# HandH1998/QQQ

Hardware: AMD Instinct MI355X
Metric: W4A8 GEMM TOPS + speedup vs fp16, M in {1..4096} N=8192 K=21760 (higher is better)
Workload: dtype i8 x i4 -> i32 -> f16; 1 GPU; qqq_gemm per-channel sweep M in {1,16,128,1024,4096} N=8192 K=21760 (configs[1]); step = the 5 calls; weights=12 rotating 89 MB int4 buffers (cold Infinity Cache), GPTQ-style N(0,0.02^2), launch=hipGraph replay, 1-step opener then 10 steps/graph, parallelism=single GPU

## Files before the change

qqq_amd/csrc/qqq_w4a8.hip:

```cpp

#include <map>
#include <mutex>
#include <thread>
#include <tuple>
#include <type_traits>
#include <utility>
#include <vector>

#include "qqq_common.hip.h"
#include "qqq_stream.hip.h"
#include "qqq_column.hip.h"
#include "qqq_panel.hip.h"
#include "qqq_tiled.hip.h"
#include "qqq_wide.hip.h"
#include "qqq_small.hip.h"
#include "qqq_act.hip.h"
#include "../../include/qqq_amd_act.h"
#include "qqq_attn.hip.h"
#include "../../include/qqq_amd_attn.h"
#include "qqq_decode.hip.h"
#include "../../include/qqq_amd_decode.h"
#include "qqq_kv8.hip.h"
#include "../../include/qqq_amd_kv8.h"
#include "qqq_paged.hip.h"
// ... 139 lines not shown
extern "C" int qqq_w4a8_model_us(int prob_m, int prob_n, int prob_k, int groupsize, int max_par, double* out) {
  g_err[0] = 0;
  if (!out || prob_m <= 0 || prob_n <= 0 || prob_k <= 0 || (prob_n % 64) != 0 || (prob_k % 64) != 0) {
    snprintf(g_err, sizeof(g_err), "qqq_w4a8_model_us: bad argument");
    return QQQ_ERR_ARG;
  }
  model_us(plan_ctx(prob_m, prob_n, prob_k, groupsize != -1, 256, max_par, true, true), out);
  return QQQ_OK;
}

extern "C" int qqq_w4a8_gemm_ex(const void* A, const void* B, void* C, void* D, const void* s1,
                                const void* s2, const void* s3, int prob_m, int prob_n, int prob_k,
                                void* workspace, int groupsize, int dev, void* stream, int thread_k,
                                int thread_n, int sms, int max_par, const qqq_tune_t* tune,
                                int32_t* acc_out, const void* bias) {
  return qqq_w4a8_gemm_ex2(A, B, C, D, s1, s2, s3, prob_m, prob_n, prob_k, workspace, groupsize, dev, stream, thread_k, thread_n, sms, max_par,
                           tune, acc_out, bias, nullptr);
}

extern "C" int qqq_w4a8_gemm_ex2(const void* A, const void* B, void* C, void* D, const void* s1,
                                 const void* s2, const void* s3, int prob_m, int prob_n, int prob_k,
                                 void* workspace, int groupsize, int dev, void* stream, int thread_k,
                                 int thread_n, int sms, int max_par, const qqq_tune_t* tune,
                                 int32_t* acc_out, const void* bias, const void* W8) {
  g_err[0] = 0;
  const int rc = ref_shape_check(prob_m, prob_n, prob_k, groupsize, thread_k, thread_n);
  if (rc != QQQ_OK) return rc;
  if (prob_m == 0 || prob_n == 0 || prob_k == 0) return QQQ_OK;
  if (!A || !B || !D || !s1 || !s2 || (groupsize != -1 && !s3)) {
    snprintf(g_err, sizeof(g_err), "null pointer argument");
    return QQQ_ERR_ARG;
  }
  if ((((uintptr_t)A | (uintptr_t)B | (uintptr_t)C | (uintptr_t)D | (uintptr_t)bias | (uintptr_t)acc_out |
        (groupsize != -1 ? (uintptr_t)s3 : 0)) & 15) != 0 ||
      (((uintptr_t)s2) & 7) != 0 || (((uintptr_t)s1 | (uintptr_t)workspace) & 3) != 0 || (((uintptr_t)W8) & 15) != 0) {
    snprintf(g_err, sizeof(g_err), "misaligned pointer argument (A/B/C/D/s3/bias/acc_out/W8: 16 bytes, s2: 8, s1/workspace: 4)");
    return QQQ_ERR_ARG;
  }
  const bool grouped = groupsize != -1;
  qqq_tune_t t;
  memset(&t, 0, sizeof(t));
  if (tune) t = *tune;
  t.w8 = (W8 != nullptr && t.w8 >= 0) ? 1 : -1;
  const int M = prob_m, N = prob_n, K = prob_k;
  int cur_dev = dev;
  if (dev < 0) (void)hipGetDevice(&cur_dev);
  const int cus_dev = device_cus_of(cur_dev);
  const bool capped = sms > 0 && sms < cus_dev;
  const PlanCtx ctx = plan_ctx(M, N, K, grouped, capped ? masked_cus(sms) : cus_dev, max_par, C != nullptr, workspace != nullptr);
  if (handoff_env_flags() & 4) t.fused |= 16;
  double est = -1.0;
  const Plan pl = make_plan(ctx, t, &est);
  if (const int M0 = choose_split(ctx, t, pl, est)) {
    qqq_tune_t tn = t;
    tn.split_m = -1;
    const int rc0 = qqq_w4a8_gemm_ex2(A, B, C, D, s1, s2, s3, M0, N, K, workspace, groupsize, dev, stream, thread_k, thread_n, sms, max_par, &tn,
                                      acc_out, bias, W8);
    if (rc0 != QQQ_OK) return rc0;
    return qqq_w4a8_gemm_ex2(static_cast<const int8_t*>(A) + (size_t)M0 * K, B, C, static_cast<_Float16*>(D) + (size_t)M0 * N,
                             static_cast<const float*>(s1) + M0, s2, s3, M - M0, N, K, workspace, groupsize, dev, stream, thread_k, thread_n, sms,
                             max_par, &tn, acc_out ? acc_out + (size_t)M0 * N : nullptr, bias, W8);
  }

  LaunchArgs a;
  a.A = static_cast<const int8_t*>(A);
  a.B = static_cast<const unsigned char*>(B);
  a.C = static_cast<int32_t*>(C);
  a.D = static_cast<_Float16*>(D);
  a.s1 = static_cast<const float*>(s1);
  a.s2 = static_cast<const float*>(s2);
  a.s3 = static_cast<const _Float16*>(s3);
  a.acc_out = acc_out;
  a.bias = static_cast<const _Float16*>(bias);
  a.tickets = static_cast<int*>(workspace);
  a.M = M;
  a.N = N;
  a.K = K;
  a.cus = ctx.cus;
  a.stream = static_cast<hipStream_t>(stream);
  a.skew = pl.skew;
  a.hflags = (pl.kernel == 2 || pl.kernel == 4 || pl.kernel == 5) ? ((t.fused >> 2) & (pl.kernel == 4 ? 15 : 7)) : 0;
  if (pl.kernel == 5 && pl.exch) a.hflags |= 8;
  if (pl.kernel == 5 && (t.fused & 128)) a.hflags |= 16;

  DeviceGuard guard(dev);
  hipError_t e = hipSuccess;
  bool reduce_launch;
  if ((pl.kernel == 1 || pl.kernel == 3 || pl.kernel == 4) && (M + 16 * pl.mt - 1) / (16 * pl.mt) > 65535) {
    snprintf(g_err, sizeof(g_err), "m=%d exceeds the grid of the small-m kernels (forced by tune)", M);
    return QQQ_ERR_ARG;
  }
  MaskedFork mf;
  if (capped) {
    hipStreamCaptureStatus cap = hipStreamCaptureStatusNone;
    if (hipStreamIsCapturing(a.stream, &cap) != hipSuccess) cap = hipStreamCaptureStatusNone;
    if (cap == hipStreamCaptureStatusNone) {
      MaskedStream* ms = masked_stream(cur_dev, sms, cus_dev, a.stream);
      if (!ms) {
        snprintf(g_err, sizeof(g_err), "sms=%d: could not create a CU-masked stream", sms);
        return QQQ_ERR_HIP;
      }
      mf.lock = std::unique_lock<std::mutex>(ms->mu);
      if ((e = hipEventRecord(ms->fork, a.stream)) != hipSuccess || (e = hipStreamWaitEvent(ms->s, ms->fork, 0)) != hipSuccess)
        return fail_hip(e, "fork into the CU-masked stream");
      mf.ms = ms;
      mf.caller = a.stream;
      a.stream = ms->s;
    }
  }
  if (pl.kernel == 5) {
    if (pl.w8) a.B = static_cast<const unsigned char*>(W8);
    e = launch_wide(a, pl.w8 ? 2 : (grouped ? 1 : 0), pl.mt, pl.bm, pl.pf, pl.pw, pl.ksplit, pl.chain != 0);
    if (e != hipSuccess) return fail_hip(e, "qqq_wide_kernel launch");
    reduce_launch = false;
  } else if (pl.kernel == 4) {
    e = launch_panel(a, grouped, pl.mt, pl.bm, pl.waves, pl.pw, pl.pf, pl.stages, pl.ksplit);
    if (e != hipSuccess) return fail_hip(e, "qqq_panel_kernel launch");
    reduce_launch = false;
  } else if (pl.kernel == 3) {
    e = launch_column(a, grouped, pl.mt, pl.pf, pl.ksplit, pl.waves);
    if (e != hipSuccess) return fail_hip(e, "qqq_column_kernel launch");
    reduce_launch = pl.ksplit > 1;
  } else if (pl.kernel == 1) {
    e = launch_stream(a, grouped, pl.mt, pl.waves, pl.pf, pl.ksplit | ((pl.fused == 3 && pl.ksplit > 1 ? pl.skew & 0xff : 0) << 16),
                      pl.ksplit > 1 ? (pl.fused == 1 ? 1 : (pl.fused == 3 ? 3 : 0)) : 0);
    if (e != hipSuccess) return fail_hip(e, "qqq_stream_kernel launch");
    reduce_launch = pl.ksplit > 1 && pl.fused != 1 && pl.fused != 3;
  } else {
    e = launch_tiled(a, grouped, pl.bm, pl.stages, pl.ksplit, pl.nslots, pl.pw);
    if (e != hipSuccess) return fail_hip(e, "qqq_tiled_kernel launch");
    reduce_launch = pl.ksplit > 1 && pl.nslots == 0;
  }
  if (reduce_launch) {
    const long long items = (long long)M * (N / 4);
    const int blocks = (int)((items + 63) / 64 > 8192 ? 8192 : (items + 63) / 64);
    hipLaunchKernelGGL(qqq_reduce_kernel, dim3(blocks), dim3(64), 0, a.stream, a.C, a.D, a.s1, a.s2,
                       a.acc_out, a.bias, M, N, pl.ksplit);
    e = hipGetLastError();
    if (e != hipSuccess) return fail_hip(e, "qqq_reduce_kernel launch");
  }
  if ((e = mf.join()) != hipSuccess) return fail_hip(e, "join from the CU-masked stream");
  return QQQ_OK;
}

extern "C" int qqq_w4a8_gemm(const void* A, const void* B, void* C, void* D, const void* s1,
                             const void* s2, const void* s3, int prob_m, int prob_n, int prob_k,
                             void* workspace, int groupsize, int dev, void* stream, int thread_k,
                             int thread_n, int sms, int max_par) {
  return qqq_w4a8_gemm_ex(A, B, C, D, s1, s2, s3, prob_m, prob_n, prob_k, workspace, groupsize, dev,
                          stream, thread_k, thread_n, sms, max_par, nullptr, nullptr, nullptr);
}

template <template <int, int> class Launch, typename... Args>
static int act_launch(const char* what, int m, int k, hipStream_t st, Args... args) {
  const int nvec = k / 8;
  const int vpt = (nvec + 255) / 256;
  if ((m <= 512 || nvec > 2048) && vpt > 2) {
    const int v4 = (nvec + 1023) / 1024;
    if (v4 <= 2)
      Launch<2, 1024>::run(m, st, args...);
    else if (v4 <= 4)
      Launch<4, 1024>::run(m, st, args...);
    else
      Launch<8, 1024>::run(m, st, args...);
  } else if (vpt <= 2)
    Launch<2, 256>::run(m, st, args...);
// ... 938 lines not shown
```

qqq_amd/csrc/qqq_wide.hip.h:

```cpp
#ifndef QQQ_AMD_QQQ_WIDE_HIP_H_
#define QQQ_AMD_QQQ_WIDE_HIP_H_


#ifndef QQQ_WIDE_ABLATE
#define QQQ_WIDE_ABLATE 0
#endif
#ifdef QQQ_PANEL_TRACE
#define QQQ_WTRV(i, v)                                                                                   \
  do {                                                                                                   \
    if (wn == 0 && qqq_trace_buf) qqq_trace_buf[(size_t)blockIdx.x * 16 + (i)] = (unsigned long long)(v); \
  } while (0)
#define QQQ_WTR(i) QQQ_WTRV(i, wall_clock64())
#else
#define QQQ_WTR(i) do {} while (0)
#define QQQ_WTRV(i, v) do {} while (0)
#endif
template <int... S, class F>
__device__ __forceinline__ void qqq_static_for(std::integer_sequence<int, S...>, F&& f) {
  (f(std::integral_constant<int, S>{}), ...);
}
template <int N, class F>
__device__ __forceinline__ void qqq_static_for(F&& f) {
  qqq_static_for(std::make_integer_sequence<int, N>{}, static_cast<F&&>(f));
}
// ... 78 lines not shown
__host__ __device__ constexpr int wide_bal_cost(int mode, int w) { return w == 0 ? 1 : (mode == 1 ? 2 : 1); }
__host__ __device__ constexpr int wide_bal_before(int mode, int mt, int hw, int t, int k, int cursors) {
  const int nslot = 2 * hw * mt, per = wide_bal_items(mode), ni = hw * per;
  int ct = 0, cb = 0, tc = 0;
  for (int j = 0; j < nslot; ++j) ct += wide_bal_cap(mode, mt, hw, t, j, cursors);
  for (int j = 0; j < k; ++j) cb += wide_bal_cap(mode, mt, hw, t, j, cursors);
  for (int i = 0; i < ni; ++i) tc += wide_bal_cost(mode, i % per);
  if (k >= nslot) return ni;
  int n = 0, e = 0;
  for (int i = 0; i < ni; ++i) {
    e += wide_bal_cost(mode, i % per);
    if ((long long)e * ct <= (long long)cb * tc) ++n;
  }
  return n;
}

template <int MODE, int MT, int HW, int T, int CURSORS>
struct WideBalTable {
  struct Tab {
    int before[2 * HW * MT + 1];
  };
  static constexpr Tab make() {
    Tab r{};
    constexpr int nslot = 2 * HW * MT, per = wide_bal_items(MODE), ni = HW * per;
    int cap[nslot] = {};
    int ct = 0, tc = 0;
    for (int j = 0; j < nslot; ++j) {
      cap[j] = wide_bal_cap(MODE, MT, HW, T, j, CURSORS);
      ct += cap[j];
    }
    for (int i = 0; i < ni; ++i) tc += wide_bal_cost(MODE, i % per);
    int cb = 0, n = 0, e = wide_bal_cost(MODE, 0);
    for (int k = 0; k < nslot; ++k) {
      while (n < ni && (long long)e * ct <= (long long)cb * tc) {
        ++n;
        if (n < ni) e += wide_bal_cost(MODE, n % per);
      }
      r.before[k] = n;
      cb += cap[k];
    }
    r.before[nslot] = ni;
    return r;
  }
  static constexpr Tab tab = make();
};

static_assert(WideBalTable<0, 16, 2, 0, 1>::tab.before[17] == wide_bal_before(0, 16, 2, 0, 17, 1) && WideBalTable<0, 16, 2, 1, 1>::tab.before[63] == wide_bal_before(0, 16, 2, 1, 63, 1) &&
                  WideBalTable<1, 8, 2, 1, 0>::tab.before[9] == wide_bal_before(1, 8, 2, 1, 9, 0) && WideBalTable<1, 16, 1, 0, 0>::tab.before[30] == wide_bal_before(1, 16, 1, 0, 30, 0),
              "the table is the function");

__host__ __device__ constexpr int wide_w8_refill_index(int mt, int hw, int k) {
  const int per = (2 * hw * mt) / (2 * hw);
  return k % per == 2 ? k / per : -1;
}
__host__ __device__ constexpr int wide_loads_in_slot(int mode, int mt, int hw, int t, int k) {
  int n = 0;
  if (mode == 1 && t == 1 && k == wide_scale_slot(hw) && !(QQQ_WIDE_ABLATE & 8)) n += 2;
  if (mode != 2 && wide_ring_load(mode, mt, hw, k) >= 0 && !(QQQ_WIDE_ABLATE & 8)) n += 1;
  if (mode == 2 && wide_w8_refill_index(mt, hw, k) >= 0 && !(QQQ_WIDE_ABLATE & 8)) n += 1;
  if (wide_dma_slot(mt, hw, k) && !(QQQ_WIDE_ABLATE & 2)) n += 1;
  return n;
}
__host__ __device__ constexpr int wide_loads_in_step(int mode, int mt, int hw, int t, int from, int to) {
  int n = 0;
  for (int k = from; k < to && k < 2 * hw * mt; ++k) n += wide_loads_in_slot(mode, mt, hw, t, k);
  return n;
}
__host__ __device__ constexpr int wide_loads_between(int mode, int mt, int hw, int t0, int k0, int steps, int k1) {
  int n = wide_loads_in_step(mode, mt, hw, t0, k0 + 1, 2 * hw * mt);
  for (int j = 1; j < steps; ++j) n += wide_loads_in_step(mode, mt, hw, (t0 + j) & 1, 0, 2 * hw * mt);
  return n + wide_loads_in_step(mode, mt, hw, (t0 + steps) & 1, 0, k1);
}
__host__ __device__ constexpr int wide_w8_last_refill_slot(int mt, int hw) {
  int last = 0;
  for (int k = 0; k < 2 * hw * mt; ++k) last = wide_w8_refill_index(mt, hw, k) >= 0 ? k : last;
  return last;
}
__host__ __device__ constexpr int wide_last_dma_slot(int mt, int hw) {
  int last = 0;
  for (int k = 0; k < 2 * hw * mt; ++k) last = wide_dma_slot(mt, hw, k) ? k : last;
  return last;
}

template <int MODE, int MT, int P, int RS, int HW, bool CHAIN = false>
__global__ __launch_bounds__(256) __attribute__((amdgpu_waves_per_eu(1, 1))) void qqq_wide_kernel(
    const int8_t* __restrict__ A, const unsigned char* __restrict__ B, int32_t* __restrict__ C, _Float16* __restrict__ D,
    const float* __restrict__ s1, const float* __restrict__ s2, const _Float16* __restrict__ s3,
    int32_t* __restrict__ acc_out, int* __restrict__ tickets, const _Float16* __restrict__ bias, const int M, const int N,
    const int K, const int tiles_m, const int tiles_n, const int PW, const int ksplit_hf) {
  const int ksplit = ksplit_hf & 0xffff, hflags = (ksplit_hf >> 16) & 0xff, skew = (ksplit_hf >> 24) & 0x3f;
  constexpr bool GROUPED = MODE == 1, W8 = MODE == 2;
  static_assert(MODE >= 0 && MODE <= 2, "0 per-channel, 1 per-group, 2 expanded int8");
  static_assert(!W8 || RS >= 3, "W8: a slot is refilled one step after its use -- RS - 1 steps of lead, the wait count needs at least one whole step in between");
  constexpr int RL = W8 ? RS - 1 : RS;
  static_assert(MT == 16 || MT == 8, "m-tiles of 16 tokens per wave (= per workgroup): 256 or 128 tokens");
  static_assert(HW == 2 || HW == 1, "a wave owns both 32-column halves of a 64-column group, or (128-column tiles) one");
  constexpr int ROWS = 16 * MT;
  constexpr int NQ = 2 * HW;
  constexpr int BN = 128 * HW;
  constexpr int NT = 256;
  constexpr int XB = ROWS * 128;
  constexpr int XPT = XB / 16 / NT;
  static_assert((2 * P) % RS == 0, "weight ring (in 64-k steps) must divide the unroll period");
  static_assert(P >= 4 && P <= 6, "LDS stage buffers: one being read, one complete, P - 2 in flight");
  constexpr int LA = P - 1;
  constexpr int NSLOT = NQ * MT;
  constexpr int EPR = HW == 2 ? 8 * MT : 16 * MT;
  constexpr int EP_STRIDE = BN + 4;

  extern __shared__ __attribute__((aligned(16))) unsigned char smem[];

  const int tid = threadIdx.x;
  const int lane = tid & 63;
  const int wn = __builtin_amdgcn_readfirstlane(tid >> 6);
  QQQ_WTR(0);

  int tile_m, tile_n, tile_lin, sp;
  auto locate = [&](const int lin, int& tm, int& tn) {
    const int full = (tiles_n / PW) * PW * tiles_m;
    if (lin < full) {
      const int panel = lin / (PW * tiles_m), within = lin % (PW * tiles_m);
      tm = within / PW;
      tn = panel * PW + within % PW;
    } else {
      const int rem = lin - full, pw = tiles_n % PW;
      tm = rem / pw;
      tn = (tiles_n / PW) * PW + rem % pw;
    }
  };
  int ch_first = 0, ch_stride = 0, ch_tiles = 1;
  {
    const int ntot = tiles_m * tiles_n * (CHAIN ? 1 : ksplit);
    const int bid = blockIdx.x;
    const int q = ntot >> 3, rr = ntot & 7;
    const int xcd = bid & 7, idx = bid >> 3;
    const int lin2 = (xcd < rr ? xcd * (q + 1) : rr * (q + 1) + (xcd - rr) * q) + idx;
    if constexpr (CHAIN) {
      const int cnt = q + (xcd < rr ? 1 : 0);
      ch_stride = (int)(gridDim.x >> 3);
      ch_first = lin2;
      ch_tiles = idx < cnt ? (cnt - idx + ch_stride - 1) / ch_stride : 0;
      if (ch_tiles == 0) return;
      sp = 0;
      tile_lin = lin2;
      locate(lin2, tile_m, tile_n);
    } else if (ksplit == 2 && (hflags & 16) != 0 && ((tiles_m * tiles_n) & 3) == 0) {
      const int per = (tiles_m * tiles_n) >> 2;
      sp = xcd & 1;
      tile_lin = (xcd >> 1) * per + idx;
      locate(tile_lin, tile_m, tile_n);
    } else {
      const int lin = lin2 / ksplit;
      sp = lin2 - lin * ksplit;
      tile_lin = lin;
      locate(lin, tile_m, tile_n);
    }
  }
  unsigned my_xcc = 0;
  if (!CHAIN && ksplit > 1) {
    asm volatile("s_getreg_b32 %0, hwreg(HW_REG_XCC_ID)" : "=s"(my_xcc));
    my_xcc &= 7u;
    if (tid == 0 && ksplit <= 6)
      __hip_atomic_fetch_or(tickets + 2 * (size_t)tile_lin, (int)((8u | my_xcc) << (8 + 4 * sp)), __ATOMIC_RELAXED, __HIP_MEMORY_SCOPE_AGENT);
  }
  const int mbase = tile_m * ROWS;
  const int ngroups = N >> 6;
  const int cb = tile_n * 4 + wn;
  int ng = HW == 2 ? cb : cb >> 1;
  const int whalf = HW == 2 ? 0 : (cb & 1);
  if (ng >= ngroups) ng = ngroups - 1;
  const unsigned rowbytes = (unsigned)N * 8u;
  const unsigned wstep = W8 ? (unsigned)N * 64u : 4u * rowbytes;
// ... 293 lines not shown
          else if constexpr (j >= 0) asm_load_w(wr[(sl + RS - 1) % RS][j], std::integral_constant<int, j>{}, swo);
        } else {
          constexpr int li = wide_dw_load_index(MT, HW, k);
          if constexpr (li >= 0) {
            if constexpr (CUR) asm_load_d(wq[sl][li / 4][li % 4], std::integral_constant<int, li>{}, cr_so, std::true_type{});
            else asm_load_d(wq[sl][li / 4][li % 4], std::integral_constant<int, li>{}, swo, std::false_type{});
          }
        }
      }
      constexpr int DP = wide_dma_period(MT, HW);
      if constexpr (wide_m0_slot(MT, HW, k) && !(QQQ_WIDE_ABLATE & 2))
        dma_m0(std::integral_constant<int, (u + LA) % P>{}, std::integral_constant<int, (XPT / 2) * t + k / DP>{});
      if constexpr (wide_dma_slot(MT, HW, k) && !(QQQ_WIDE_ABLATE & 2)) {
        if constexpr (CUR) dma_go_cur(std::integral_constant<int, (XPT / 2) * t + k / DP>{});
        else dma_go(std::integral_constant<int, (XPT / 2) * t + k / DP>{}, st_xso);
      }
      if constexpr (t == 1 && k == BSLOT) {
        constexpr int since = wide_loads_between(MODE, MT, HW, 1, wide_last_dma_slot(MT, HW), 2 * (P - 3), k + 1);
        static_assert(since < 64, "vmcnt is a 6-bit counter");
        if constexpr (!(QQQ_WIDE_ABLATE & 1)) asm volatile("s_waitcnt vmcnt(%0)\n\ts_barrier" : : "n"(since) : "memory");
        else asm volatile("s_waitcnt vmcnt(%0)" : : "n"(since) : "memory");
      }
      __builtin_amdgcn_sched_barrier(0);
    };
    qqq_static_for<NSLOT>(slot);
  };

  constexpr int SCB = ROWS * 4 + BN * 6;
  constexpr int SC0 = P * XB;
  const int cej = lane & 15, cecp = lane >> 4;
  const int cegrp = HW == 2 ? wn : (wn >> 1), cehalf = wn & 1;
  auto scale_dma = [&](const int tm, const int tn, const int par) __attribute__((always_inline)) {
    const unsigned voff = (unsigned)((64 * wn + lane) * 4);
    const int rows = M - tm * ROWS < ROWS ? M - tm * ROWS : ROWS, cols = N - tn * BN < BN ? N - tn * BN : BN;
    auto one = [&](const void* base, const unsigned bytes, const unsigned dst) {
      v4u d = descriptor(base);
      d[2] = (unsigned)__builtin_amdgcn_readfirstlane((int)bytes);
      const unsigned m0v = (unsigned)__builtin_amdgcn_readfirstlane((int)dst);
      asm volatile("s_mov_b32 m0, %2\n\ts_nop 4\n\tbuffer_load_dword %0, %1, 0 offen lds" : : "v"(voff), "s"(d), "s"(m0v) : "memory");
    };
    const unsigned r0 = (unsigned)(SC0 + par * SCB + 256 * wn);
    if (wn < ROWS / 64) one(s1 + (size_t)tm * ROWS, (unsigned)rows * 4u, r0);
    if (wn < BN / 64) one(s2 + (size_t)tn * BN, (unsigned)cols * 4u, r0 + ROWS * 4);
    if (wn < BN / 128 && bias) one(bias + (size_t)tn * BN, (unsigned)cols * 2u, r0 + ROWS * 4 + BN * 4);
  };
  auto flush_tile = [&](const int tm, const int tn, const int par) __attribute__((always_inline)) {
    asm volatile("s_nop 15\n\ts_nop 15" ::: "memory");
    const unsigned char* sc = smem + SC0 + par * SCB;
    const float* s1t = reinterpret_cast<const float*>(sc);
    const float* s2t = reinterpret_cast<const float*>(sc + ROWS * 4);
    const _Float16* bt = reinterpret_cast<const _Float16*>(sc + ROWS * 4 + BN * 4);
    const _Float16 nzc = (_Float16)-0.0f;
    const int cl = 64 * cegrp + 16 * cecp;
    const bool cols_ok = tn * BN + 64 * cegrp < N;
    float2 dsa[NQ], dsb[NQ];
    h4 dbv[NQ];
    int dl[NQ];
#pragma unroll
    for (int q = 0; q < NQ; ++q) {
      dl[q] = cl + 8 * (q & 1) + 4 * (HW == 2 ? (q >> 1) : cehalf);
      const int i0 = s2_stored_index(dl[q]);
      dsa[q] = *reinterpret_cast<const float2*>(s2t + i0);
      dsb[q] = *reinterpret_cast<const float2*>(s2t + i0 + 8);
      dbv[q] = (h4){nzc, nzc, nzc, nzc};
    }
    if (bias) {
#pragma unroll
      for (int q = 0; q < NQ; ++q) dbv[q] = *reinterpret_cast<const h4*>(bt + dl[q]);
    }
    v4i zero4 = {0, 0, 0, 0};
    asm volatile("" : "+v"(zero4));
    const int rows = M - tm * ROWS < ROWS ? M - tm * ROWS : ROWS;
    const __amdgpu_buffer_rsrc_t dview = __builtin_amdgcn_make_buffer_rsrc(D + (size_t)tm * ROWS * N, 0, rows * N * 2, 0x00020000);
    const __amdgpu_buffer_rsrc_t aview = __builtin_amdgcn_make_buffer_rsrc(acc_out ? acc_out + (size_t)tm * ROWS * N : (int32_t*)D, 0, rows * N * 4, 0x00020000);
    const unsigned drow = (unsigned)(cej * N + tn * BN) * 2u;
#pragma unroll
    for (int mt = 0; mt < MT; ++mt) {
      const float ts = s1t[16 * mt + cej];
      h4 o[NQ];
#pragma unroll
      for (int q = 0; q < NQ; q += 2) {
        v4i ra = acc[mt][q], rb = acc[mt][q + 1];
        asm volatile("" : "+v"(ra), "+v"(rb));
        asm volatile("v_mfma_i32_16x16x64_i8 %0, %1, %1, 0" : "+a"(acc[mt][q]) : "v"(zero4));
        asm volatile("v_mfma_i32_16x16x64_i8 %0, %1, %1, 0" : "+a"(acc[mt][q + 1]) : "v"(zero4));
        int a0 = ra[0], a1 = ra[1], a2 = ra[2], a3 = ra[3], b0 = rb[0], b1 = rb[1], b2 = rb[2], b3 = rb[3];
        asm volatile("s_nop 1\n\t"
                     "v_permlane16_swap_b32 %0, %1\n\tv_permlane16_swap_b32 %2, %3\n\t"
                     "v_permlane16_swap_b32 %4, %5\n\tv_permlane16_swap_b32 %6, %7\n\t"
                     "v_permlane32_swap_b32 %0, %2\n\tv_permlane32_swap_b32 %1, %3\n\t"
                     "v_permlane32_swap_b32 %4, %6\n\tv_permlane32_swap_b32 %5, %7"
                     : "+v"(a0), "+v"(a1), "+v"(a2), "+v"(a3), "+v"(b0), "+v"(b1), "+v"(b2), "+v"(b3));
        if (acc_out && cols_ok) {
          const unsigned ar = (drow + (unsigned)(16 * mt) * (unsigned)N * 2u) * 2u;
          __builtin_amdgcn_raw_buffer_store_b128((v4u){(unsigned)a0, (unsigned)a1, (unsigned)a2, (unsigned)a3}, aview, ar + (unsigned)dl[q] * 4u, 0, 0);
          __builtin_amdgcn_raw_buffer_store_b128((v4u){(unsigned)b0, (unsigned)b1, (unsigned)b2, (unsigned)b3}, aview, ar + (unsigned)dl[q + 1] * 4u, 0, 0);
        }
        o[q] = epilogue_vals4(a0, a1, a2, a3, ts, dsa[q], dsb[q]) + dbv[q];
        o[q + 1] = epilogue_vals4(b0, b1, b2, b3, ts, dsa[q + 1], dsb[q + 1]) + dbv[q + 1];
      }
      if (cols_ok) {
        const unsigned dr = drow + (unsigned)(16 * mt) * (unsigned)N * 2u;
        if constexpr (HW == 2) {
          const h8 lo8 = {o[0][0], o[0][1], o[0][2], o[0][3], o[2][0], o[2][1], o[2][2], o[2][3]};
          const h8 hi8 = {o[1][0], o[1][1], o[1][2], o[1][3], o[3][0], o[3][1], o[3][2], o[3][3]};
          __builtin_amdgcn_raw_buffer_store_b128(__builtin_bit_cast(v4u, lo8), dview, dr + (unsigned)cl * 2u, 0, 0);
          __builtin_amdgcn_raw_buffer_store_b128(__builtin_bit_cast(v4u, hi8), dview, dr + (unsigned)cl * 2u + 16u, 0, 0);
        } else {
          typedef unsigned v2u __attribute__((ext_vector_type(2)));
#pragma unroll
          for (int q = 0; q < NQ; ++q) __builtin_amdgcn_raw_buffer_store_b64(__builtin_bit_cast(v2u, o[q]), dview, dr + (unsigned)dl[q] * 2u, 0, 0);
        }
      }
      __builtin_amdgcn_sched_barrier(0);
    }
  };
  auto seam = [&]() __attribute__((always_inline)) {
    QQQ_WTRV(ch_pos < 7 ? 2 + 2 * ch_pos : 15, wall_clock64());
    flush_tile(cur_tm, cur_tn, ch_pos & 1);
    QQQ_WTRV(ch_pos < 7 ? 3 + 2 * ch_pos : 15, wall_clock64());
    ++ch_pos;
    cur_tm = nx_tm, cur_tn = nx_tn;
    cu_a_lo = nx_a_lo, cu_a_hi = nx_a_hi, cu_a_rec = nx_a_rec, cu_w_so = nx_w_so, cu_s_so = nx_s_so;
    if (ch_pos < ch_tiles) {
      scale_dma(cur_tm, cur_tn, ch_pos & 1);
      if (ch_pos + 1 < ch_tiles) locate(ch_first + (ch_pos + 1) * ch_stride, nx_tm, nx_tn);
      nx_tm = __builtin_amdgcn_readfirstlane(nx_tm), nx_tn = __builtin_amdgcn_readfirstlane(nx_tn);
      tile_ref(nx_tm, nx_tn, nx_a_lo, nx_a_hi, nx_a_rec, nx_w_so, nx_s_so);
    }
    cursors_at_stage0();
  };

  constexpr int RST = NT / (BN / 8);
  const int c8 = tid % (BN / 8), er0 = tid / (BN / 8);
  const int n = tile_n * BN + c8 * 8;
  float2 s2v[4] = {};
  const _Float16 nz = (_Float16)-0.0f;
  h8 bv = {nz, nz, nz, nz, nz, nz, nz, nz};
  if (!CHAIN && n < N) {
    const int i0s = s2_stored_index(n), i1s = s2_stored_index(n + 4);
    s2v[0] = *reinterpret_cast<const float2*>(s2 + i0s);
    s2v[1] = *reinterpret_cast<const float2*>(s2 + i0s + 8);
    s2v[2] = *reinterpret_cast<const float2*>(s2 + i1s);
    s2v[3] = *reinterpret_cast<const float2*>(s2 + i1s + 8);
    if (bias) bv = *reinterpret_cast<const h8*>(bias + n);
  }

  if constexpr (CHAIN) {
    scale_dma(tile_m, tile_n, 0);
    qqq_static_for<LA>([&](auto jc) { dma_stage_so(jc, (unsigned)decltype(jc)::value * 128u); });
#pragma unroll
    for (int j = 0; j < RL; ++j) {
      if constexpr (DW) load_d_step(cu_w_so + (unsigned)j * wstep, wq[j]);
      else load_w_so(cu_w_so + (unsigned)j * wstep, wr[j]);
    }
    if constexpr (GROUPED) {
#pragma unroll
      for (int j = 0; j < P; ++j) load_sc_so(cu_s_so + (unsigned)j * (unsigned)N * 2u, scr[j]);
    }
  } else {
    qqq_static_for<LA>([&](auto jc) { dma_stage(jc, decltype(jc)::value); });
#pragma unroll
    for (int j = 0; j < RL; ++j) {
      if constexpr (DW) load_d_step((unsigned)(2 * st0 + (j < KS ? j : KS - 1)) * wstep, wq[j]);
      else load_w(j, wr[j]);
    }
    if constexpr (GROUPED) {
#pragma unroll
      for (int j = 0; j < P; ++j) load_sc(j, scr[j]);
    }
  }
  qqq_static_for<RL>([&](auto jc) {
    constexpr int j = decltype(jc)::value;
    (void)wr[0];
    if constexpr (DW) {
      (void)wq[0][0][0];
      qqq_static_for<HW>([&](auto hfc) {
        constexpr int hf = decltype(hfc)::value;
        (void)wq[0][0][0];
        asm volatile("s_waitcnt vmcnt(0)" : "+v"(wq[j][hf][0]), "+v"(wq[j][hf][1]), "+v"(wq[j][hf][2]), "+v"(wq[j][hf][3]));
      });
    } else if constexpr (HW == 2) asm volatile("s_waitcnt vmcnt(0)" : "+v"(wr[j][0]), "+v"(wr[j][1]), "+v"(wr[j][2]), "+v"(wr[j][3]));
    else asm volatile("s_waitcnt vmcnt(0)" : "+v"(wr[j][0]), "+v"(wr[j][1]));
  });
  if constexpr (GROUPED) {
    qqq_static_for<P>([&](auto jc) {
      (void)scr[0];
      asm volatile("" : "+v"(scr[decltype(jc)::value][0]), "+v"(scr[decltype(jc)::value][1]));
    });
  }
  __syncthreads();
#pragma unroll
  for (int mt = 0; mt < MT; ++mt) read_x(0, 0, mt);
  if constexpr (!W8) {
    qqq_static_for<HW>([&](auto hfc) {
      constexpr int hf = decltype(hfc)::value;
      un_setup(__builtin_bit_cast(h2, scr[0][hf]));
      (void)wq[0][0][0];
      qqq_static_for<UPARTS>([&](auto pc) { un_part(pc, hfc, aop[0], wq[0][hf]); });
    });
  }
  __builtin_amdgcn_sched_barrier(0);

  if constexpr (CUR) {
    cx_so = sgpr((unsigned)(st0 + LA - 1) * 128u);
    cr_so = sgpr((unsigned)(2 * st0 + RL) * wstep);
    cc_so = sgpr((unsigned)(st0 + P) * (unsigned)N * 2u);
  }
  auto do_stage = [&](const int i, auto uc) __attribute__((always_inline)) {
    step(i, uc, std::integral_constant<int, 0>{});
    step(i, uc, std::integral_constant<int, 1>{});
  };
  QQQ_WTR(1);
  if constexpr (CHAIN) {
    static_assert(!CHAIN || P == 4, "the trip is written out for four stage buffers");
    int left = NST;
    auto do_stage_chain = [&](auto uc) __attribute__((always_inline)) {
      const unsigned sstep = (unsigned)N * 2u;
      if (__builtin_expect(left > P, 1)) {
        st_xso = sgpr(cx_so), st_swo[0] = sgpr(cr_so), st_swo[1] = sgpr(cr_so + wstep), st_sco = sgpr(cc_so);
        cx_so += 128u, cr_so += 2u * wstep, cc_so += sstep;
        asm volatile("" : "+s"(st_xso), "+s"(st_swo[0]), "+s"(st_swo[1]), "+s"(st_sco));
      } else {
        const int done = NST - left;
        const bool xn = left <= LA, cn = true;
        st_xso = sgpr(xn ? (unsigned)(LA - left) * 128u : (unsigned)(done + LA) * 128u);
        xdesc[0] = sgpr(xn ? nx_a_lo : cu_a_lo), xdesc[1] = sgpr(xn ? nx_a_hi : cu_a_hi), xdesc[2] = sgpr(xn ? nx_a_rec : cu_a_rec);
#pragma unroll
        for (int t = 0; t < 2; ++t) {
          const int sn_ = 2 * done + t + RL;
          st_swo[t] = sgpr(sn_ < KS ? cu_w_so + (unsigned)sn_ * wstep : nx_w_so + (unsigned)(sn_ - KS) * wstep);
        }
        st_sco = sgpr(cn ? nx_s_so + (unsigned)(P - left) * sstep : 0u);
        asm volatile("s_nop 4" : "+s"(st_xso), "+s"(st_swo[0]), "+s"(st_swo[1]), "+s"(st_sco), "+s"(xdesc));
      }
      step(0, uc, std::integral_constant<int, 0>{});
      step(0, uc, std::integral_constant<int, 1>{});
    };
    bool more = true;
#define QQQ_CHAIN_STAGE(U)                                    \
  if (__builtin_expect(more, 1)) {                            \
    do_stage_chain(std::integral_constant<int, U>{});         \
    if (__builtin_expect(--left == 0, 0)) {                   \
      seam();                                                 \
      left = NST;                                             \
      if (ch_pos == ch_tiles) {                               \
        asm volatile("s_waitcnt vmcnt(0)" ::: "memory");      \
        more = false;                                         \
      }                                                       \
    }                                                         \
  }
    do {
      QQQ_CHAIN_STAGE(0)
      QQQ_CHAIN_STAGE(1)
      QQQ_CHAIN_STAGE(2)
      QQQ_CHAIN_STAGE(3)
    } while (more);
    return;
#undef QQQ_CHAIN_STAGE
  }
  int i0 = 0;
  for (; i0 + P <= NST; i0 += P) {
#if defined(QQQ_PANEL_TRACE) && defined(QQQ_WIDE_TRACE_TRIPS)
    if (i0 < 12 * P) QQQ_WTRV(4 + i0 / P, __builtin_amdgcn_s_memtime());
#endif
    qqq_static_for<P>([&](auto uc) __attribute__((always_inline)) { do_stage(i0 + decltype(uc)::value, uc); });
  }
  qqq_static_for<P - 1>([&](auto uc) __attribute__((always_inline)) {
    if (i0 + decltype(uc)::value < NST) do_stage(i0 + decltype(uc)::value, uc);
  });

  asm volatile("s_waitcnt vmcnt(0)" ::: "memory");
  if constexpr (DW) {
    qqq_static_for<RS * HW>([&](auto jc) {
      constexpr int j = decltype(jc)::value / HW, hf = decltype(jc)::value % HW;
      (void)wq[0][0][0];
      asm volatile("" : : "v"(wq[j][hf][0]), "v"(wq[j][hf][1]), "v"(wq[j][hf][2]), "v"(wq[j][hf][3]));
    });
  }
  qqq_static_for<RS>([&](auto jc) {
    (void)wr[0];
    if constexpr (DW) return;
    asm volatile("" : : "v"(wr[decltype(jc)::value][0]), "v"(wr[decltype(jc)::value][WRN - 1]));
    if constexpr (W8 && HW == 2) asm volatile("" : : "v"(wr[decltype(jc)::value][1]), "v"(wr[decltype(jc)::value][2]));
  });
  if constexpr (GROUPED) {
    qqq_static_for<P>([&](auto jc) {
      (void)scr[0];
      asm volatile("" : : "v"(scr[decltype(jc)::value][0]), "v"(scr[decltype(jc)::value][1]));
    });
  }
  QQQ_WTR(2);
  asm volatile("s_nop 15\n\ts_nop 15" ::: "memory");
  int* ep = reinterpret_cast<int*>(smem);
  const int ej = lane & 15, ecp = lane >> 4;
  const int egrp = HW == 2 ? wn : (wn >> 1), ehalf = wn & 1;
  constexpr int EP_ITEMS = EPR * (BN / 8), EP_PASSES = EP_ITEMS / NT;
  auto image = [&](const int pass) __attribute__((always_inline)) {
#pragma unroll
    for (int jm = 0; jm < EPR / 16; ++jm)
#pragma unroll
      for (int q = 0; q < NQ; ++q)
#pragma unroll
        for (int r = 0; r < 4; ++r)
          ep[(16 * jm + ej) * EP_STRIDE + 64 * egrp + 16 * r + 8 * (q & 1) + 4 * (HW == 2 ? (q >> 1) : ehalf) + ecp] = acc[pass * (EPR / 16) + jm][q][r];
  };

  constexpr unsigned XB_EXCH = 1u << 16, XB_CLASSIC = 1u << 17;
  const bool exch_on = ksplit == 2 && (hflags & 8) != 0 && ROWS / EPR == 2;
  int arrival = 0;
  bool exch = false;
  if (ksplit > 1) {
    int* tk = tickets + 2 * (size_t)tile_lin;
    int* xch = ep + EPR * EP_STRIDE;
    if (tid == 0) {
      unsigned w = (unsigned)__hip_atomic_fetch_add(tk, 1, __ATOMIC_RELAXED, __HIP_MEMORY_SCOPE_AGENT);
      if (exch_on) {
        const unsigned arr = w & 0xffu;
        if (arr == 0) {
          const unsigned dec = (((w >> (8 + 4 * (1 - sp))) & 8u) != 0) ? XB_EXCH : XB_CLASSIC;
          (void)__hip_atomic_fetch_or(tk, (int)dec, __ATOMIC_RELAXED, __HIP_MEMORY_SCOPE_AGENT);
          w |= dec;
        } else {
          int spin = 0;
          while (!(w & (XB_EXCH | XB_CLASSIC))) {
            if (++spin > QQQ_SPIN_LIMIT) __builtin_trap();
            __builtin_amdgcn_s_sleep(1);
            w = (unsigned)__hip_atomic_load(tk, __ATOMIC_RELAXED, __HIP_MEMORY_SCOPE_AGENT);
          }
          w = (w & ~0xffu) | arr;
        }
      }
      *xch = (int)w;
    }
    __syncthreads();
    const unsigned word = (unsigned)__builtin_amdgcn_readfirstlane(*xch);
    arrival = (int)(word & 0xffu);
    exch = exch_on && (word & XB_EXCH) != 0;
#ifndef QQQ_WIDE_TRACE_TRIPS
    QQQ_WTR(4);
    QQQ_WTRV(7, (arrival << 1) | (exch ? 1 : 0));
#endif
    const size_t slot_ints = (size_t)ROWS * BN;
    if (exch || arrival < ksplit - 1) {
      bool local = ksplit <= 6 && !(hflags & 4);
      for (int j = 0; j < ksplit; ++j) local = local && ((word >> (8 + 4 * j)) & 15u) == (8u | my_xcc);
      const __amdgpu_buffer_rsrc_t sv = wide_view(C + ((size_t)tile_lin * (ksplit - 1) + (exch ? 0 : arrival)) * slot_ints);
      auto deposit = [&](auto auxc) __attribute__((always_inline)) {
        constexpr int aux = decltype(auxc)::value;
#pragma unroll
        for (int pass = 0; pass < ROWS / EPR; ++pass) {
          if (exch && pass == sp) continue;
          __syncthreads();
          image(pass);
          __syncthreads();
#pragma unroll
          for (int ps = 0; ps < EP_PASSES; ++ps) {
            const int row = er0 + RST * ps;
            const unsigned off = (unsigned)(((pass * EPR + row) * BN + c8 * 8) * 4);
            const v4i lo = *reinterpret_cast<const v4i*>(ep + row * EP_STRIDE + c8 * 8);
            const v4i hi4 = *reinterpret_cast<const v4i*>(ep + row * EP_STRIDE + c8 * 8 + 4);
            __builtin_amdgcn_raw_buffer_store_b128(__builtin_bit_cast(v4u, lo), sv, off, 0, aux);
            __builtin_amdgcn_raw_buffer_store_b128(__builtin_bit_cast(v4u, hi4), sv, off + 16, 0, aux);
          }
        }
      };
      if (local) deposit(std::integral_constant<int, 0>{});
      else deposit(std::integral_constant<int,  17>{});
      asm volatile("s_waitcnt vmcnt(0)" ::: "memory");
      __syncthreads();
      if (tid == 0) qqq_publish_add(tk + 1, hflags);
#ifndef QQQ_WIDE_TRACE_TRIPS
      QQQ_WTR(5);
#endif
// ... 23 lines not shown
    }
    if (folding) {
      for (int sl = 0; sl < ksplit - 1; ++sl) {
        const __amdgpu_buffer_rsrc_t sv = agent_view(slots + (size_t)sl * ((size_t)ROWS * BN));
        v4i d0[RB], d1[RB];
#pragma unroll
        for (int j = 0; j < RB; ++j) {
          const unsigned off = (unsigned)(((pass * EPR + er0 + RST * (half * RB + j)) * BN + c8 * 8) * 4);
          d0[j] = load16_agent(sv, off);
          d1[j] = load16_agent(sv, off + 16);
        }
#pragma unroll
        for (int j = 0; j < RB; ++j) {
          lo[j] += d0[j];
          hi4[j] += d1[j];
        }
      }
    }
#pragma unroll
    for (int j = 0; j < RB; ++j) {
      const int ps = half * RB + j;
      const int m = mbase + pass * EPR + er0 + RST * ps;
      const h4 o0 = epilogue_vals4(lo[j][0], lo[j][1], lo[j][2], lo[j][3], a_s[pass][ps], s2v[0], s2v[1]);
      const h4 o1 = epilogue_vals4(hi4[j][0], hi4[j][1], hi4[j][2], hi4[j][3], a_s[pass][ps], s2v[2], s2v[3]);
      h8 o = {o0[0], o0[1], o0[2], o0[3], o1[0], o1[1], o1[2], o1[3]};
      o = o + bv;
      if (!guarded || (m < M && n < N)) {
        *reinterpret_cast<h8*>(D + (size_t)m * N + n) = o;
        if (guarded && acc_out) {
          *reinterpret_cast<v4i*>(acc_out + (size_t)m * N + n) = lo[j];
          *reinterpret_cast<v4i*>(acc_out + (size_t)m * N + n + 4) = hi4[j];
        }
      }
    }
  };
  const int first_pass = exch ? sp : 0;
#pragma unroll
  for (int pass = 0; pass < ROWS / EPR; ++pass) {
    if (exch && pass != sp) continue;
    __syncthreads();
    image(pass);
    if (pass == first_pass && fold) {
      if (tid == 0) {
        int* tk = tickets + 2 * (size_t)tile_lin;
        int spin = 0;
        while (__hip_atomic_load(tk + 1, __ATOMIC_RELAXED, __HIP_MEMORY_SCOPE_AGENT) < (exch ? 2 : ksplit - 1)) {
          if (++spin > QQQ_SPIN_LIMIT) __builtin_trap();
          __builtin_amdgcn_s_sleep(2);
        }
        if (!exch || __hip_atomic_fetch_add(tk + 1, 1, __ATOMIC_RELAXED, __HIP_MEMORY_SCOPE_AGENT) == 3) {
          __hip_atomic_store(tk, 0, __ATOMIC_RELAXED, __HIP_MEMORY_SCOPE_AGENT);
          __hip_atomic_store(tk + 1, 0, __ATOMIC_RELAXED, __HIP_MEMORY_SCOPE_AGENT);
        }
      }
    }
    __syncthreads();
#ifndef QQQ_WIDE_TRACE_TRIPS
    if (pass == first_pass && fold) QQQ_WTR(6);
#endif
    if (pass == first_pass && fold && qqq_formal_acquire(hflags)) __builtin_amdgcn_fence(__ATOMIC_ACQUIRE, "agent");
    if (pass == first_pass) {
#pragma unroll
      for (int p2 = 0; p2 < ROWS / EPR; ++p2)
#pragma unroll
        for (int ps = 0; ps < EP_PASSES; ++ps) asm volatile("" : "+v"(a_s[p2][ps]));
    }
    if (interior && !fold) {
#pragma unroll
      for (int hb = 0; hb < EP_PASSES / RB; ++hb) out_rows(pass, hb, false, false);
    } else if (interior) {
#pragma unroll
      for (int hb = 0; hb < EP_PASSES / RB; ++hb) out_rows(pass, hb, false, true);
    } else {
#pragma unroll
      for (int hb = 0; hb < EP_PASSES / RB; ++hb) out_rows(pass, hb, true, fold);
    }
  }
#ifdef QQQ_PANEL_TRACE
  asm volatile("s_waitcnt vmcnt(0)" ::: "memory");
  QQQ_WTR(3);
#endif
}

template <int MODE, int MT, int P, int RS, int HW, bool CHAIN = false>
static hipError_t launch_wide_t(const LaunchArgs& a, int pw, int ksplit) {
  constexpr int ROWS = 16 * MT, BN = 128 * HW;
  constexpr int XBUF = P * ROWS * 128, EP = (HW == 2 ? 8 * MT : 16 * MT) * (BN + 4) * 4 + 16;
  constexpr int CH = XBUF + 2 * (ROWS * 4 + BN * 6);
  constexpr int LDS = CHAIN ? CH : (XBUF > EP ? XBUF : EP);
  static_assert(LDS <= 160 * 1024, "LDS budget");
  static bool attr_set[64] = {};
  auto kern = qqq_wide_kernel<MODE, MT, P, RS, HW, CHAIN>;
  if (hipError_t e = allow_dynamic_lds(kern, LDS, attr_set); e != hipSuccess) return e;
  const int tiles_m = (a.M + ROWS - 1) / ROWS, tiles_n = (a.N + BN - 1) / BN;
  const int grid = CHAIN ? (a.cus & ~7) : tiles_m * tiles_n * ksplit;
  hipLaunchKernelGGL(kern, dim3(grid), dim3(256), LDS, a.stream, a.A, a.B, a.C, a.D, a.s1, a.s2, a.s3,
                     a.acc_out, a.tickets, a.bias, a.M, a.N, a.K, tiles_m, tiles_n, pw,
                     ksplit | ((a.hflags & 0xff) << 16) | ((!CHAIN && ksplit > 1 ? a.skew & 0x3f : 0) << 24));
  return hipGetLastError();
}

template <int MODE, int MT>
static hipError_t launch_wide_m(const LaunchArgs& a, int pf, int pw, int ksplit) {
  return pf == 4 ? launch_wide_t<MODE, MT, 4, 4, 2>(a, pw, ksplit) : launch_wide_t<MODE, MT, 4, 8, 2>(a, pw, ksplit);
}
static hipError_t launch_wide_chain(const LaunchArgs& a, int mode, int mt, int bn, int pw) {
  if (mode == 2) return launch_wide_t<2, 16, 4, 4, 2, true>(a, pw, 1);
  const bool grouped = mode == 1;
  if (bn == 128) return grouped ? launch_wide_t<1, 16, 4, 4, 1, true>(a, pw, 1) : launch_wide_t<0, 16, 4, 4, 1, true>(a, pw, 1);
  if (mt == 8) return grouped ? launch_wide_t<1, 8, 4, 4, 2, true>(a, pw, 1) : launch_wide_t<0, 8, 4, 4, 2, true>(a, pw, 1);
  return grouped ? launch_wide_t<1, 16, 4, 4, 2, true>(a, pw, 1) : launch_wide_t<0, 16, 4, 4, 2, true>(a, pw, 1);
}
static hipError_t launch_wide(const LaunchArgs& a, int mode, int mt, int bn, int pf, int pw, int ksplit, bool chain = false) {
  if (chain) return launch_wide_chain(a, mode, mt, bn, pw);
  if (mode == 2) {
    if (bn == 128) return launch_wide_t<2, 16, 4, 4, 1>(a, pw, ksplit);
    if (mt == 8) return launch_wide_t<2, 8, 4, 4, 2>(a, pw, ksplit);
    return launch_wide_t<2, 16, 4, 4, 2>(a, pw, ksplit);
  }
  const bool grouped = mode == 1;
  if (bn == 128) {
    if (grouped) return pf == 4 ? launch_wide_t<1, 16, 4, 4, 1>(a, pw, ksplit) : launch_wide_t<1, 16, 4, 8, 1>(a, pw, ksplit);
    return pf == 4 ? launch_wide_t<0, 16, 4, 4, 1>(a, pw, ksplit) : launch_wide_t<0, 16, 4, 8, 1>(a, pw, ksplit);
  }
  if (mt == 8) return grouped ? launch_wide_m<1, 8>(a, pf, pw, ksplit) : launch_wide_m<0, 8>(a, pf, pw, ksplit);
  return grouped ? launch_wide_m<1, 16>(a, pf, pw, ksplit) : launch_wide_m<0, 16>(a, pf, pw, ksplit);
}

#endif
```

Before: 2895 TOPS.

## Add flush variant of wide kernel reusing chain-style epilogue for non-split tiles

Adds a FLUSH instantiation of the wide kernel, launched automatically for evenly divisible shapes with no k-split and no accumulator output. It loads the scales by DMA into LDS and writes the output through the chain kernel's flush_tile path, replacing the separate LDS-staged epilogue. It also skips the accumulator-zeroing MFMAs and acc_out stores outside the chain kernel. A tune flag bit (hflags 32) can switch the path off, and the flush kernel uses a different LDS size, which may change occupancy or introduce correctness risks.

```diff
diff --git a/qqq_amd/csrc/qqq_w4a8.hip b/qqq_amd/csrc/qqq_w4a8.hip
--- a/qqq_amd/csrc/qqq_w4a8.hip
+++ b/qqq_amd/csrc/qqq_w4a8.hip
@@ -245,6 +245,7 @@
   a.hflags = (pl.kernel == 2 || pl.kernel == 4 || pl.kernel == 5) ? ((t.fused >> 2) & (pl.kernel == 4 ? 15 : 7)) : 0;
   if (pl.kernel == 5 && pl.exch) a.hflags |= 8;
   if (pl.kernel == 5 && (t.fused & 128)) a.hflags |= 16;
+  if (pl.kernel == 5 && (t.fused & 256)) a.hflags |= 32;
 
   DeviceGuard guard(dev);
   hipError_t e = hipSuccess;
diff --git a/qqq_amd/csrc/qqq_wide.hip.h b/qqq_amd/csrc/qqq_wide.hip.h
--- a/qqq_amd/csrc/qqq_wide.hip.h
+++ b/qqq_amd/csrc/qqq_wide.hip.h
@@ -184,12 +184,13 @@
   return last;
 }
 
-template <int MODE, int MT, int P, int RS, int HW, bool CHAIN = false>
-__global__ __launch_bounds__(256) __attribute__((amdgpu_waves_per_eu(1, 1))) void qqq_wide_kernel(
+template <int MODE, int MT, int P, int RS, int HW, bool CHAIN, bool FLUSH>
+__device__ __forceinline__ void qqq_wide_body(
     const int8_t* __restrict__ A, const unsigned char* __restrict__ B, int32_t* __restrict__ C, _Float16* __restrict__ D,
     const float* __restrict__ s1, const float* __restrict__ s2, const _Float16* __restrict__ s3,
     int32_t* __restrict__ acc_out, int* __restrict__ tickets, const _Float16* __restrict__ bias, const int M, const int N,
     const int K, const int tiles_m, const int tiles_n, const int PW, const int ksplit_hf) {
+  static_assert(!(CHAIN && FLUSH), "the walk has its own seams");
   const int ksplit = ksplit_hf & 0xffff, hflags = (ksplit_hf >> 16) & 0xff, skew = (ksplit_hf >> 24) & 0x3f;
   constexpr bool GROUPED = MODE == 1, W8 = MODE == 2;
   static_assert(MODE >= 0 && MODE <= 2, "0 per-channel, 1 per-group, 2 expanded int8");
@@ -649,8 +650,10 @@
       for (int q = 0; q < NQ; q += 2) {
         v4i ra = acc[mt][q], rb = acc[mt][q + 1];
         asm volatile("" : "+v"(ra), "+v"(rb));
-        asm volatile("v_mfma_i32_16x16x64_i8 %0, %1, %1, 0" : "+a"(acc[mt][q]) : "v"(zero4));
-        asm volatile("v_mfma_i32_16x16x64_i8 %0, %1, %1, 0" : "+a"(acc[mt][q + 1]) : "v"(zero4));
+        if constexpr (CHAIN) {
+          asm volatile("v_mfma_i32_16x16x64_i8 %0, %1, %1, 0" : "+a"(acc[mt][q]) : "v"(zero4));
+          asm volatile("v_mfma_i32_16x16x64_i8 %0, %1, %1, 0" : "+a"(acc[mt][q + 1]) : "v"(zero4));
+        }
         int a0 = ra[0], a1 = ra[1], a2 = ra[2], a3 = ra[3], b0 = rb[0], b1 = rb[1], b2 = rb[2], b3 = rb[3];
         asm volatile("s_nop 1\n\t"
                      "v_permlane16_swap_b32 %0, %1\n\tv_permlane16_swap_b32 %2, %3\n\t"
@@ -658,7 +661,7 @@
                      "v_permlane32_swap_b32 %0, %2\n\tv_permlane32_swap_b32 %1, %3\n\t"
                      "v_permlane32_swap_b32 %4, %6\n\tv_permlane32_swap_b32 %5, %7"
                      : "+v"(a0), "+v"(a1), "+v"(a2), "+v"(a3), "+v"(b0), "+v"(b1), "+v"(b2), "+v"(b3));
-        if (acc_out && cols_ok) {
+        if (CHAIN && acc_out && cols_ok) {
           const unsigned ar = (drow + (unsigned)(16 * mt) * (unsigned)N * 2u) * 2u;
           __builtin_amdgcn_raw_buffer_store_b128((v4u){(unsigned)a0, (unsigned)a1, (unsigned)a2, (unsigned)a3}, aview, ar + (unsigned)dl[q] * 4u, 0, 0);
           __builtin_amdgcn_raw_buffer_store_b128((v4u){(unsigned)b0, (unsigned)b1, (unsigned)b2, (unsigned)b3}, aview, ar + (unsigned)dl[q + 1] * 4u, 0, 0);
@@ -704,7 +707,7 @@
   float2 s2v[4] = {};
   const _Float16 nz = (_Float16)-0.0f;
   h8 bv = {nz, nz, nz, nz, nz, nz, nz, nz};
-  if (!CHAIN && n < N) {
+  if (!CHAIN && !FLUSH && n < N) {
     const int i0s = s2_stored_index(n), i1s = s2_stored_index(n + 4);
     s2v[0] = *reinterpret_cast<const float2*>(s2 + i0s);
     s2v[1] = *reinterpret_cast<const float2*>(s2 + i0s + 8);
@@ -726,6 +729,7 @@
       for (int j = 0; j < P; ++j) load_sc_so(cu_s_so + (unsigned)j * (unsigned)N * 2u, scr[j]);
     }
   } else {
+    if constexpr (FLUSH) scale_dma(tile_m, tile_n, 0);
     qqq_static_for<LA>([&](auto jc) { dma_stage(jc, decltype(jc)::value); });
 #pragma unroll
     for (int j = 0; j < RL; ++j) {
@@ -837,26 +841,36 @@
     if (i0 + decltype(uc)::value < NST) do_stage(i0 + decltype(uc)::value, uc);
   });
 
-  asm volatile("s_waitcnt vmcnt(0)" ::: "memory");
-  if constexpr (DW) {
-    qqq_static_for<RS * HW>([&](auto jc) {
-      constexpr int j = decltype(jc)::value / HW, hf = decltype(jc)::value % HW;
-      (void)wq[0][0][0];
-      asm volatile("" : : "v"(wq[j][hf][0]), "v"(wq[j][hf][1]), "v"(wq[j][hf][2]), "v"(wq[j][hf][3]));
+  auto drain_loads = [&]() __attribute__((always_inline)) {
+    asm volatile("s_waitcnt vmcnt(0)" ::: "memory");
+    if constexpr (DW) {
+      qqq_static_for<RS * HW>([&](auto jc) {
+        constexpr int j = decltype(jc)::value / HW, hf = decltype(jc)::value % HW;
+        (void)wq[0][0][0];
+        asm volatile("" : : "v"(wq[j][hf][0]), "v"(wq[j][hf][1]), "v"(wq[j][hf][2]), "v"(wq[j][hf][3]));
+      });
+    }
+    qqq_static_for<RS>([&](auto jc) {
+      (void)wr[0];
+      if constexpr (DW) return;
+      asm volatile("" : : "v"(wr[decltype(jc)::value][0]), "v"(wr[decltype(jc)::value][WRN - 1]));
+      if constexpr (W8 && HW == 2) asm volatile("" : : "v"(wr[decltype(jc)::value][1]), "v"(wr[decltype(jc)::value][2]));
     });
-  }
-  qqq_static_for<RS>([&](auto jc) {
-    (void)wr[0];
-    if constexpr (DW) return;
-    asm volatile("" : : "v"(wr[decltype(jc)::value][0]), "v"(wr[decltype(jc)::value][WRN - 1]));
-    if constexpr (W8 && HW == 2) asm volatile("" : : "v"(wr[decltype(jc)::value][1]), "v"(wr[decltype(jc)::value][2]));
-  });
-  if constexpr (GROUPED) {
-    qqq_static_for<P>([&](auto jc) {
-      (void)scr[0];
-      asm volatile("" : : "v"(scr[decltype(jc)::value][0]), "v"(scr[decltype(jc)::value][1]));
-    });
-  }
+    if constexpr (GROUPED) {
+      qqq_static_for<P>([&](auto jc) {
+        (void)scr[0];
+        asm volatile("" : : "v"(scr[decltype(jc)::value][0]), "v"(scr[decltype(jc)::value][1]));
+      });
+    }
+  };
+  if constexpr (FLUSH) {
+    QQQ_WTR(2);
+    flush_tile(tile_m, tile_n, 0);
+    drain_loads();
+    QQQ_WTR(3);
+    return;
+  }
+  drain_loads();
   QQQ_WTR(2);
   asm volatile("s_nop 15\n\ts_nop 15" ::: "memory");
   int* ep = reinterpret_cast<int*>(smem);
@@ -1046,15 +1060,31 @@
 #endif
 }
 
+#define QQQ_WIDE_ARGS                                                                                                     \
+  const int8_t *__restrict__ A, const unsigned char *__restrict__ B, int32_t *__restrict__ C, _Float16 *__restrict__ D,   \
+      const float *__restrict__ s1, const float *__restrict__ s2, const _Float16 *__restrict__ s3, int32_t *__restrict__ acc_out, \
+      int *__restrict__ tickets, const _Float16 *__restrict__ bias, const int M, const int N, const int K, const int tiles_m,     \
+      const int tiles_n, const int PW, const int ksplit_hf
 template <int MODE, int MT, int P, int RS, int HW, bool CHAIN = false>
+__global__ __launch_bounds__(256) __attribute__((amdgpu_waves_per_eu(1, 1))) void qqq_wide_kernel(QQQ_WIDE_ARGS) {
+  qqq_wide_body<MODE, MT, P, RS, HW, CHAIN, false>(A, B, C, D, s1, s2, s3, acc_out, tickets, bias, M, N, K, tiles_m, tiles_n, PW, ksplit_hf);
+}
+template <int MODE, int MT, int P, int RS, int HW>
+__global__ __launch_bounds__(256) __attribute__((amdgpu_waves_per_eu(1, 1))) void qqq_wide_flush_kernel(QQQ_WIDE_ARGS) {
+  qqq_wide_body<MODE, MT, P, RS, HW, false, true>(A, B, C, D, s1, s2, s3, acc_out, tickets, bias, M, N, K, tiles_m, tiles_n, PW, ksplit_hf);
+}
+#undef QQQ_WIDE_ARGS
+
+template <int MODE, int MT, int P, int RS, int HW, bool CHAIN = false, bool FLUSH = false>
 static hipError_t launch_wide_t(const LaunchArgs& a, int pw, int ksplit) {
   constexpr int ROWS = 16 * MT, BN = 128 * HW;
   constexpr int XBUF = P * ROWS * 128, EP = (HW == 2 ? 8 * MT : 16 * MT) * (BN + 4) * 4 + 16;
   constexpr int CH = XBUF + 2 * (ROWS * 4 + BN * 6);
-  constexpr int LDS = CHAIN ? CH : (XBUF > EP ? XBUF : EP);
+  constexpr int LDS = CHAIN ? CH : FLUSH ? XBUF + (ROWS * 4 + BN * 6) : (XBUF > EP ? XBUF : EP);
   static_assert(LDS <= 160 * 1024, "LDS budget");
   static bool attr_set[64] = {};
   auto kern = qqq_wide_kernel<MODE, MT, P, RS, HW, CHAIN>;
+  if constexpr (FLUSH) kern = qqq_wide_flush_kernel<MODE, MT, P, RS, HW>;
   if (hipError_t e = allow_dynamic_lds(kern, LDS, attr_set); e != hipSuccess) return e;
   const int tiles_m = (a.M + ROWS - 1) / ROWS, tiles_n = (a.N + BN - 1) / BN;
   const int grid = CHAIN ? (a.cus & ~7) : tiles_m * tiles_n * ksplit;
@@ -1075,8 +1105,19 @@
   if (mt == 8) return grouped ? launch_wide_t<1, 8, 4, 4, 2, true>(a, pw, 1) : launch_wide_t<0, 8, 4, 4, 2, true>(a, pw, 1);
   return grouped ? launch_wide_t<1, 16, 4, 4, 2, true>(a, pw, 1) : launch_wide_t<0, 16, 4, 4, 2, true>(a, pw, 1);
 }
+static bool wide_flush_applies(const LaunchArgs& a, int mt, int bn, int pf, int ksplit) {
+  return pf == 4 && ksplit == 1 && a.acc_out == nullptr && !(a.hflags & 32) && a.M % (16 * mt) == 0 && a.N % bn == 0;
+}
+template <int MODE>
+static hipError_t launch_wide_flush(const LaunchArgs& a, int mt, int bn, int pw) {
+  if (bn == 128) return launch_wide_t<MODE, 16, 4, 4, 1, false, true>(a, pw, 1);
+  if (mt == 8) return launch_wide_t<MODE, 8, 4, 4, 2, false, true>(a, pw, 1);
+  return launch_wide_t<MODE, 16, 4, 4, 2, false, true>(a, pw, 1);
+}
 static hipError_t launch_wide(const LaunchArgs& a, int mode, int mt, int bn, int pf, int pw, int ksplit, bool chain = false) {
   if (chain) return launch_wide_chain(a, mode, mt, bn, pw);
+  if (wide_flush_applies(a, mt, bn, mode == 2 ? 4 : pf, ksplit))
+    return mode == 2 ? launch_wide_flush<2>(a, mt, bn, pw) : mode == 1 ? launch_wide_flush<1>(a, mt, bn, pw) : launch_wide_flush<0>(a, mt, bn, pw);
   if (mode == 2) {
     if (bn == 128) return launch_wide_t<2, 16, 4, 4, 1>(a, pw, ksplit);
     if (mt == 8) return launch_wide_t<2, 8, 4, 4, 2>(a, pw, ksplit);
```

After: 2926 TOPS, median of 6. +1.0%, better.
